# WU-CVGL/DreamMesh4D

Measured on AMD Instinct MI355X. Metric: rendered views/sec (fwd+bwd, 512^2, 200k Gaussians), higher is better.
Workload: dtype f32

## Files before the change

### dreammesh4d_amd/csrc/raster_preprocess.hip

```cpp
#include "common.h"
#include "raster.h"

#ifndef DM4D_GREC
#define DM4D_GREC 128
#endif
namespace dm4d {

struct f3 { float x, y, z; };

__device__ __forceinline__ f3 xform4x3(const f3 p, const float *M)
{
    f3 o;
    o.x = ((M[0] * p.x + M[4] * p.y) + M[8] * p.z) + M[12];
    o.y = ((M[1] * p.x + M[5] * p.y) + M[9] * p.z) + M[13];
    o.z = ((M[2] * p.x + M[6] * p.y) + M[10] * p.z) + M[14];
    return o;
}
__device__ __forceinline__ float4 xform4x4(const f3 p, const float *M)
{
    float4 o;
    o.x = ((M[0] * p.x + M[4] * p.y) + M[8] * p.z) + M[12];
    o.y = ((M[1] * p.x + M[5] * p.y) + M[9] * p.z) + M[13];
    o.z = ((M[2] * p.x + M[6] * p.y) + M[10] * p.z) + M[14];
    o.w = ((M[3] * p.x + M[7] * p.y) + M[11] * p.z) + M[15];
// ... 52 lines not shown
    float J02 = -(vp.focal_x * tcx) / (t.z * t.z);
    float J11 = vp.focal_y / t.z;
    float J12 = -(vp.focal_y * tcy) / (t.z * t.z);
    float T0[3], T1[3];
#pragma unroll
    for (int j = 0; j < 3; ++j) {
        T0[j] = J00 * V[j * 4 + 0] + J02 * V[j * 4 + 2];
        T1[j] = J11 * V[j * 4 + 1] + J12 * V[j * 4 + 2];
    }
    const float S[9] = {cov6[0], cov6[1], cov6[2], cov6[1], cov6[3], cov6[4], cov6[2], cov6[4], cov6[5]};
    float v0[3], v1[3];
#pragma unroll
    for (int j = 0; j < 3; ++j) {
        v0[j] = (T0[0] * S[0 * 3 + j] + T0[1] * S[1 * 3 + j]) + T0[2] * S[2 * 3 + j];
        v1[j] = (T1[0] * S[0 * 3 + j] + T1[1] * S[1 * 3 + j]) + T1[2] * S[2 * 3 + j];
    }
    c[0] = (v0[0] * T0[0] + v0[1] * T0[1]) + v0[2] * T0[2];
    c[1] = (v0[0] * T1[0] + v0[1] * T1[1]) + v0[2] * T1[2];
    c[2] = (v1[0] * T1[0] + v1[1] * T1[1]) + v1[2] * T1[2];
    if (aux) {
#pragma unroll
        for (int j = 0; j < 3; ++j) { aux->T0[j] = T0[j]; aux->T1[j] = T1[j]; }
        aux->tz = t.z;
        aux->tcx = tcx;
        aux->tcy = tcy;
        aux->xclamped = (txtz < -limx || txtz > limx);
        aux->yclamped = (tytz < -limy || tytz > limy);
    }
}

#define DM4D_SH_C0 0.28209479177387814f

__device__ __forceinline__ f3 load3(const float *p, int i) { return f3{p[3 * i], p[3 * i + 1], p[3 * i + 2]}; }

__global__ __launch_bounds__(kPreThreads) void k_preprocess(BatchDesc d)
{
    extern __shared__ __attribute__((aligned(16))) uint32_t s_hist[];
    const ViewCtx c = resolve(d, blockIdx.y);
    const ViewParams &vp = c.vp;
    const dm4d_raster_inputs &in = c.in;
    int32_t *__restrict__ radii = c.radii;
    const GeomPtrs &g = c.g;
    const int T = c.T;
    __shared__ float sV[16], sP[16];
    __shared__ uint32_t s_wsum[2][kPreThreads / 64];
    const int tid = threadIdx.x;
    if (tid < 16) { sV[tid] = vp.view[tid]; sP[tid] = vp.proj[tid]; }
    for (int t = tid; t < T; t += kPreThreads) s_hist[t] = 0u;
    __syncthreads();
    uint32_t touched_sum = 0, rec_sum = 0;
#pragma unroll 1
    for (int it = 0; it < kPreItems; ++it) {
        const int i = blockIdx.x * kPreBlock + it * kPreThreads + tid;
        if (i >= in.N) break;
        uint32_t touched = 0, recs = 0;
        int my_radius = 0;
        const f3 p = load3(in.means3D, i);
        const f3 pv = xform4x3(p, sV);
        if (pv.z > 0.2f) {
            const float4 ph = xform4x4(p, sP);
            const float pw = 1.0f / (ph.w + 0.0000001f);
            const float ppx = ph.x * pw, ppy = ph.y * pw;
            float cov6[6];
            if (in.cov3D_precomp) {
#pragma unroll
                for (int k = 0; k < 6; ++k) cov6[k] = in.cov3D_precomp[6 * (size_t)i + k];
            } else {
                const float4 q = reinterpret_cast<const float4 *>(in.rotations)[i];
                cov3d_from_scale_rot(load3(in.scales, i), vp.scale_modifier, q, cov6);
            }
            float c[3];
            cov2d(p, vp, sV, cov6, c, nullptr);
            c[0] += 0.3f;
            c[2] += 0.3f;
            const float det = c[0] * c[2] - c[1] * c[1];
            if (det != 0.0f) {
                const float det_inv = 1.f / det;
                const float mid = 0.5f * (c[0] + c[2]);
                const float disc = sqrtf(fmaxf(0.1f, mid * mid - det));
                const float lambda1 = mid + disc, lambda2 = mid - disc;
                const int r = f2i_sat(ceilf(3.f * sqrtf(fmaxf(lambda1, lambda2))));
                const float px = ((ppx + 1.0f) * (float)vp.W - 1.0f) * 0.5f;
                const float py = ((ppy + 1.0f) * (float)vp.H - 1.0f) * 0.5f;
                const Rect rc = tile_rect(px, py, r, vp.gx, vp.gy);
                const int area = (rc.x1 - rc.x0) * (rc.y1 - rc.y0);
                if (area != 0) {
                    my_radius = r;
                    touched = (uint32_t)area;
                    g.xy[i] = make_float2(px, py);
                    g.depth[i] = pv.z;
                    const float4 co = make_float4(c[2] * det_inv, -c[1] * det_inv, c[0] * det_inv, in.opacities[i]);
                    g.conic_opacity[i] = co;
                    const Bands bd = cell_bands(px, py, co.x, co.y, co.z, co.w, rc);
                    recs = (uint32_t)(bd.nbx * bd.nby);
                    uint32_t dense = 1u;
                    const float cdet = co.x * co.z - co.y * co.y;
                    if (bd.nbx >= 2 && bd.nby >= 2 && recs <= 64u && cdet > 0.f && co.x > 0.f && co.z > 0.f) {
                        const float tau = __logf(255.0f * co.w) * 1.001f + 0.01f;
                        const EllipseRows er = ellipse_rows(co.x, co.y, co.z, tau);
                        uint64_t mask = 0ull;
                        for (int by = 0; by < bd.nby; ++by) {
                            int b0, b1;
                            row_span(er, px, py, (float)(4 * (bd.by0 + by)), b0, b1);
                            b0 = max(b0 - bd.bx0, 0);
                            b1 = min(b1 - bd.bx0, bd.nbx - 1);
                            if (b0 <= b1) mask |= ((~0ull >> (63 - (b1 - b0))) << b0) << (by * bd.nbx);
                        }
                        g.cellmask[i] = mask;
                        recs = (uint32_t)__popcll(mask);
                        dense = 0u;
                    }
                    g.cellinfo[i] = make_uint4((uint32_t)bd.bx0 | ((uint32_t)bd.by0 << 16),
                                               (uint32_t)bd.nbx | ((uint32_t)bd.nby << 16), 0u, dense);
                    if (d.tile_records) {
                        const TileSpan ts = tile_span((uint32_t)bd.bx0 | ((uint32_t)bd.by0 << 16), (uint32_t)bd.nbx | ((uint32_t)bd.nby << 16));
                        recs = (uint32_t)(ts.tnx * ts.tny);
                    }
                    if (in.shs) {
                        const float *sh = in.shs + (size_t)i * in.sh_coeffs * 3;
#pragma unroll
                        for (int ch = 0; ch < 3; ++ch) {
                            float v = DM4D_SH_C0 * sh[ch] + 0.5f;
                            g.clamped[3 * (size_t)i + ch] = (v < 0.f);
                            g.rgb[3 * (size_t)i + ch] = fmaxf(v, 0.f);
                        }
                    }
                    for (int y = rc.y0; y < rc.y1; ++y)
                        for (int x = rc.x0; x < rc.x1; ++x) atomicAdd(&s_hist[y * vp.gx + x], 1u);
                }
            }
        }
        radii[i] = my_radius;
        g.tiles_touched[i] = touched;
        g.rec_touched[i] = recs;
        touched_sum += touched;
        rec_sum += recs;
    }
    const uint32_t ws = wave_sum_u32(touched_sum), wr = wave_sum_u32(rec_sum);
    if ((tid & 63) == 0) { s_wsum[0][tid >> 6] = ws; s_wsum[1][tid >> 6] = wr; }
    __syncthreads();
    uint32_t *row = g.hist + (size_t)blockIdx.x * T;
    for (int t = tid; t < T; t += kPreThreads) row[t] = s_hist[t];
    if (tid == 0) {
        uint32_t s = 0, r = 0;
#pragma unroll
        for (int w = 0; w < kPreThreads / 64; ++w) { s += s_wsum[0][w]; r += s_wsum[1][w]; }
        g.block_sums[blockIdx.x] = s;
        g.rec_block_sums[blockIdx.x] = r;
        if (s) atomicAdd(&g.counters[kCntD], s);
        if (r) atomicAdd(&g.counters[kCntR], r);
    }
}

__device__ __forceinline__ uint32_t block_excl_scan_256(uint32_t v, uint32_t *s_w , uint32_t *total)
{
    const int tid = threadIdx.x, lane = tid & 63, wv = tid >> 6;
    const uint32_t incl = wave_incl_scan_u32(v, lane);
    __syncthreads();
    if (lane == 63) s_w[wv] = incl;
    __syncthreads();
    uint32_t pre = 0, tot = 0;
#pragma unroll
    for (int w = 0; w < kPreThreads / 64; ++w) {
        const uint32_t x = s_w[w];
        if (w < wv) pre += x;
        tot += x;
    }
    *total = tot;
    return pre + incl - v;
}

__global__ __launch_bounds__(kPreThreads) void k_scatter(BatchDesc d)
{
    extern __shared__ __attribute__((aligned(16))) uint32_t s_cursor[];
    const ViewCtx c = resolve(d, blockIdx.y);
    const ViewParams &vp = c.vp;
    const int N = c.in.N, T = c.T;
    const int32_t *__restrict__ radii = c.radii;
    const GeomPtrs &g = c.g;
    const BinPtrs &b = c.b;
    const uint32_t cap = c.cap;
    __shared__ uint32_t s_w[kPreThreads / 64];
    const int tid = threadIdx.x;
    {
        const int per = (T + kPreThreads - 1) / kPreThreads;
        const int t0 = tid * per, t1 = min(T, t0 + per);
        uint32_t loc = 0;
        for (int t = t0; t < t1; ++t) loc += g.tile_count[t];
        uint32_t total;
        uint32_t run = block_excl_scan_256(loc, s_w, &total);
        const uint32_t *row = g.hist + (size_t)blockIdx.x * T;
        for (int t = t0; t < t1; ++t) {
            if (blockIdx.x == 0) g.tile_start[t] = run;
            s_cursor[t] = run + row[t];
            run += g.tile_count[t];
        }
        if (blockIdx.x == 0 && tid == 0) g.tile_start[T] = total;
    }
    if (blockIdx.x == 0) {
        __shared__ uint32_t s_oh[256], s_oc[256], s_omax;
        if (tid == 0) s_omax = 1u;
        s_oh[tid] = 0u;
        __syncthreads();
        uint32_t wmax = 0;
        for (int t = tid; t < T; t += kPreThreads) wmax = max(wmax, g.tile_count[t]);
        wmax = wave_max_u32(wmax);
        if ((tid & 63) == 0) atomicMax(&s_omax, wmax);
        __syncthreads();
        const float oscale = 255.0f / (float)s_omax;
        for (int t = tid; t < T; t += kPreThreads)
            atomicAdd(&s_oh[255 - min(255, (int)((float)g.tile_count[t] * oscale))], 1u);
        __syncthreads();
        if (tid == 0) {
            uint32_t run = 0;
            for (int k = 0; k < 256; ++k) { s_oc[k] = run; run += s_oh[k]; }
        }
        __syncthreads();
        for (int t = tid; t < T; t += kPreThreads)
            g.order[atomicAdd(&s_oc[255 - min(255, (int)((float)g.tile_count[t] * oscale))], 1u)] = (uint32_t)t;
    }
    uint32_t rcarry;
    {
        uint32_t rloc = 0;
        for (int w = tid; w < (int)blockIdx.x; w += kPreThreads) rloc += g.rec_block_sums[w];
        uint32_t total;
        block_excl_scan_256(rloc, s_w, &total);
        rcarry = total;
    }
    __syncthreads();
    bool overflow = false, rec_overflow = false;
#pragma unroll 1
    for (int it = 0; it < kPreItems; ++it) {
        const int i = blockIdx.x * kPreBlock + it * kPreThreads + tid;
        const uint32_t touched = (i < N) ? g.tiles_touched[i] : 0u;
        uint32_t total;
        const uint32_t recs = (i < N) ? g.rec_touched[i] : 0u;
        const uint32_t r0 = rcarry + block_excl_scan_256(recs, s_w, &total);
        rcarry += total;
        if (i < N && touched != 0u) {
            reinterpret_cast<uint32_t *>(g.cellinfo + i)[2] = r0;
            g.rec0[i] = r0;
            rec_overflow |= (recs > 0u) && ((uint64_t)r0 + recs > (uint64_t)c.rec_cap);
        }
        if (touched == 0) continue;
        const float2 xy = g.xy[i];
        const Rect rc = tile_rect(xy.x, xy.y, radii[i], vp.gx, vp.gy);
        const uint32_t dbits = __float_as_uint(g.depth[i]);
        uint32_t n = 0;
        for (int y = rc.y0; y < rc.y1; ++y)
            for (int x = rc.x0; x < rc.x1; ++x, ++n) {
                const uint32_t slot = atomicAdd(&s_cursor[y * vp.gx + x], 1u);
                if (slot < cap) {
                    b.u_depth[slot] = dbits;
                    b.u_idx[slot] = (uint32_t)i;
                } else {
                    overflow = true;
                }
            }
    }
    if (overflow) g.counters[kCntOverflow] = 1u;
    if (rec_overflow) g.counters[kCntRecOverflow] = 1u;
}

struct GatherOut { float dmean[3], drot[4], dcol[kMaxChannels]; };

constexpr int kGatherRecords(int parts) { return parts <= 3 ? DM4D_GREC : 96; }
template <int PARTS>
__device__ __forceinline__ void gather_gaussian(const BatchDesc &d, const ViewCtx &c, const int i, const bool live, const float *sV,
                                                const float *sP, float *chunk, GatherOut &res)
{
    const ViewParams &vp = c.vp;
    const dm4d_raster_inputs &in = c.in;
    const int32_t *__restrict__ radii = c.radii;
    const GeomPtrs &g = c.g;
    const float *__restrict__ dLt = c.dLq;
    const BwdOutputs &o = c.o;
    constexpr int kGRec = kGatherRecords(PARTS), kGStride = PARTS <= 3 ? 12 : 20;
    constexpr int NQ = kGRec * PARTS / 64;
    const int lane = threadIdx.x & 63;
    const size_t si = (size_t)i;
#pragma unroll
    for (int k = 0; k < 3; ++k) res.dmean[k] = 0.f;
#pragma unroll
    for (int k = 0; k < 4; ++k) res.drot[k] = 0.f;
#pragma unroll
    for (int k = 0; k < kMaxChannels; ++k) res.dcol[k] = 0.f;

    float acc[7 + kMaxChannels];
#pragma unroll
    for (int k = 0; k < 7 + kMaxChannels; ++k) acc[k] = 0.f;
    const int r = live ? radii[i] : 0;
    const int C = vp.C;
    f3 h_m = {0.f, 0.f, 0.f}, h_sc = {0.f, 0.f, 0.f};
    float4 h_q = make_float4(1.f, 0.f, 0.f, 0.f), h_co = make_float4(0.f, 0.f, 0.f, 0.f);
    if (r > 0) {
        h_m = load3(in.means3D, i);
        if (!in.cov3D_precomp) { h_q = reinterpret_cast<const float4 *>(in.rotations)[i]; h_sc = load3(in.scales, i); }
        h_co = g.conic_opacity[i];
    }
    {
        const bool lean = d.lean != 0;
        constexpr int RS = PARTS * 4;
        uint32_t rec0 = 0xFFFFFFFFu, end = 0u;
        if (r > 0) {
            const uint32_t cnt = g.rec_touched[i];
            if (cnt > 0u) {
                rec0 = g.cellinfo[i].z;
                end = min(rec0 + cnt, max(rec0, c.rec_cap));
            }
        }
        uint32_t R0 = rec0, R1 = end;
        R0 = wave_min_u32(R0);
        R1 = wave_max_u32(R1);
        float4 pq[NQ];
#pragma unroll
        for (int q = 0; q < NQ; ++q) pq[q] = make_float4(0.f, 0.f, 0.f, 0.f);
#define DM4D_FETCH(BASE)                                                                                   \
        {                                                                                                  \
            const uint32_t n4_ = min((uint32_t)kGRec, R1 - (BASE)) * (uint32_t)PARTS;                      \
            const float4 *src4_ = reinterpret_cast<const float4 *>(dLt + (size_t)(BASE) * RS);             \
            _Pragma("unroll") for (int q = 0; q < NQ; ++q)                                                 \
                if ((uint32_t)lane + 64u * q < n4_) pq[q] = src4_[lane + 64 * q];                          \
        }
        if (R0 < R1) DM4D_FETCH(R0)
        for (uint32_t base = R0; base < R1; base += kGRec) {
            const uint32_t nrec = min((uint32_t)kGRec, R1 - base);
            __builtin_amdgcn_wave_barrier();
#pragma unroll
            for (int q = 0; q < NQ; ++q) {
                const uint32_t idx4 = (uint32_t)lane + 64u * q;
                if (idx4 < nrec * (uint32_t)PARTS)
                    *reinterpret_cast<float4 *>(chunk + (idx4 / (uint32_t)PARTS) * kGStride + (idx4 % (uint32_t)PARTS) * 4) = pq[q];
            }
            if (base + kGRec < R1) DM4D_FETCH(base + kGRec)
            __builtin_amdgcn_wave_barrier();
            const uint32_t lo = max(rec0, base), hi = min(end, base + nrec);
            for (uint32_t slot = lo; slot < hi; ++slot) {
                const float4 *rp = reinterpret_cast<const float4 *>(chunk + (slot - base) * kGStride);
                const float4 a0 = rp[0], a1 = rp[1];
                acc[0] += a0.x; acc[1] += a0.y; acc[2] += a0.z; acc[3] += a0.w;
                if (PARTS == 2) {
                    acc[4] += a1.x; acc[10] += a1.y; acc[11] += a1.z; acc[12] += a1.w;
                    continue;
                }
                const float4 a2 = rp[2];
                if (lean) {
                    acc[4] += a1.x; acc[6] += a1.y; acc[10] += a1.z; acc[11] += a1.w; acc[12] += a2.x;
                    continue;
                }
                acc[4] += a1.x; acc[5] += a1.y; acc[6] += a1.z; acc[7] += a1.w;
                acc[8] += a2.x; acc[9] += a2.y;
                if (C > 3) {
                    const float4 a3 = rp[3];
                    acc[10] += a2.z; acc[11] += a2.w; acc[12] += a3.x;
                }
            }
        }
#undef DM4D_FETCH
    }
    {
        const float4 co = h_co;
        const float m0 = acc[0], m1 = acc[1];
        acc[0] = -(co.x * m0 + co.y * m1) * (0.5f * (float)vp.W);
        acc[1] = -(co.y * m0 + co.z * m1) * (0.5f * (float)vp.H);
        acc[2] = -0.5f * acc[2];
        acc[3] = -acc[3];
        acc[4] = -0.5f * acc[4];
    }
    if (!live) return;
    if (o.dL_dmeans2D) {
        o.dL_dmeans2D[3 * si + 0] = acc[0];
        o.dL_dmeans2D[3 * si + 1] = acc[1];
        o.dL_dmeans2D[3 * si + 2] = 0.f;
    }
#pragma unroll
    for (int ch = 0; ch < kMaxChannels; ++ch) res.dcol[ch] = acc[7 + ch];
    if (o.dL_dopacity) {
        const float op_ = in.opacities[i];
        o.dL_dopacity[si] = (r > 0 && op_ > 0.f) ? acc[5] / op_ : 0.f;
    }
    if (o.dL_dcolors) {
        for (int ch = 0; ch < C; ++ch) o.dL_dcolors[(size_t)C * si + ch] = acc[7 + ch];
    }
    if (o.dL_dsh && in.shs) {
        const int M = in.sh_coeffs;
        for (int ch = 0; ch < 3; ++ch)
            o.dL_dsh[si * M * 3 + ch] = (r > 0 && !g.clamped[3 * si + ch]) ? DM4D_SH_C0 * acc[7 + ch] : 0.f;
        for (int k = 3; k < 3 * M; ++k) o.dL_dsh[si * M * 3 + k] = 0.f;
    }

    float dmean[3] = {0.f, 0.f, 0.f};
    float dcov[6] = {0.f, 0.f, 0.f, 0.f, 0.f, 0.f};
    float dscale[3] = {0.f, 0.f, 0.f};
    float drot[4] = {0.f, 0.f, 0.f, 0.f};
    if (r > 0) {
        const f3 m = h_m;
        float cov6[6];
        float4 q = make_float4(1.f, 0.f, 0.f, 0.f);
        f3 sc = {0.f, 0.f, 0.f};
        if (in.cov3D_precomp) {
#pragma unroll
            for (int k = 0; k < 6; ++k) cov6[k] = in.cov3D_precomp[6 * si + k];
        } else {
            q = h_q; sc = h_sc;
            cov3d_from_scale_rot(sc, vp.scale_modifier, q, cov6);
        }
        float c[3];
        Cov2DAux aux;
        cov2d(m, vp, sV, cov6, c, &aux);
        const float a = c[0] + 0.3f, bb = c[1], cc = c[2] + 0.3f;
        const float denom = a * cc - bb * bb;
        const float denom2inv = 1.0f / ((denom * denom) + 0.0000001f);
        const float gA = acc[2], gB = acc[3], gC = acc[4];
        float dL_da = 0.f, dL_db = 0.f, dL_dc = 0.f;
        const float *T0 = aux.T0, *T1 = aux.T1;
        if (denom2inv != 0.f) {
            dL_da = denom2inv * (-cc * cc * gA + bb * cc * gB + (denom - a * cc) * gC);
            dL_dc = denom2inv * (-a * a * gC + a * bb * gB + (denom - a * cc) * gA);
            dL_db = denom2inv * (2 * bb * cc * gA - (denom + 2 * bb * bb) * gB + 2 * a * bb * gC);
            dcov[0] = T0[0] * T0[0] * dL_da + T0[0] * T1[0] * dL_db + T1[0] * T1[0] * dL_dc;
            dcov[3] = T0[1] * T0[1] * dL_da + T0[1] * T1[1] * dL_db + T1[1] * T1[1] * dL_dc;
            dcov[5] = T0[2] * T0[2] * dL_da + T0[2] * T1[2] * dL_db + T1[2] * T1[2] * dL_dc;
            dcov[1] = 2 * T0[0] * T0[1] * dL_da + (T0[0] * T1[1] + T0[1] * T1[0]) * dL_db + 2 * T1[0] * T1[1] * dL_dc;
            dcov[2] = 2 * T0[0] * T0[2] * dL_da + (T0[0] * T1[2] + T0[2] * T1[0]) * dL_db + 2 * T1[0] * T1[2] * dL_dc;
            dcov[4] = 2 * T0[2] * T0[1] * dL_da + (T0[1] * T1[2] + T0[2] * T1[1]) * dL_db + 2 * T1[1] * T1[2] * dL_dc;
        }
        {
            const float S[9] = {cov6[0], cov6[1], cov6[2], cov6[1], cov6[3], cov6[4], cov6[2], cov6[4], cov6[5]};
            float dT0[3], dT1[3];
#pragma unroll
            for (int k = 0; k < 3; ++k) {
                const float s0 = S[k * 3 + 0] * T0[0] + S[k * 3 + 1] * T0[1] + S[k * 3 + 2] * T0[2];
                const float s1 = S[k * 3 + 0] * T1[0] + S[k * 3 + 1] * T1[1] + S[k * 3 + 2] * T1[2];
                dT0[k] = 2 * s0 * dL_da + s1 * dL_db;
                dT1[k] = 2 * s1 * dL_dc + s0 * dL_db;
            }
            float dJ00 = 0, dJ02 = 0, dJ11 = 0, dJ12 = 0;
#pragma unroll
            for (int k = 0; k < 3; ++k) {
                dJ00 += sV[k * 4 + 0] * dT0[k];
                dJ02 += sV[k * 4 + 2] * dT0[k];
                dJ11 += sV[k * 4 + 1] * dT1[k];
                dJ12 += sV[k * 4 + 2] * dT1[k];
            }
            const float tz = 1.f / aux.tz, tz2 = tz * tz, tz3 = tz2 * tz;
            const float xm = aux.xclamped ? 0.f : 1.f, ym = aux.yclamped ? 0.f : 1.f;
            const float fx = vp.focal_x, fy = vp.focal_y;
            const float dtx = xm * -fx * tz2 * dJ02;
            const float dty = ym * -fy * tz2 * dJ12;
            const float dtz = -fx * tz2 * dJ00 - fy * tz2 * dJ11 + (2 * fx * aux.tcx) * tz3 * dJ02 +
                              (2 * fy * aux.tcy) * tz3 * dJ12;
#pragma unroll
            for (int j = 0; j < 3; ++j) dmean[j] = sV[j * 4 + 0] * dtx + sV[j * 4 + 1] * dty + sV[j * 4 + 2] * dtz;
        }
        {
            const float4 ph = xform4x4(m, sP);
            const float mw = 1.0f / (ph.w + 0.0000001f);
            const float mul1 = ph.x * mw * mw, mul2 = ph.y * mw * mw;
#pragma unroll
            for (int j = 0; j < 3; ++j)
                dmean[j] += (sP[j * 4 + 0] * mw - sP[j * 4 + 3] * mul1) * acc[0] +
                            (sP[j * 4 + 1] * mw - sP[j * 4 + 3] * mul2) * acc[1];
        }
        {
            const float mul3 = sV[2] * m.x + sV[6] * m.y + sV[10] * m.z + sV[14];
#pragma unroll
            for (int j = 0; j < 3; ++j) dmean[j] += (sV[j * 4 + 2] - sV[j * 4 + 3] * mul3) * acc[6];
        }
        if (!in.cov3D_precomp) {
            float R[9];
            quat_to_R(q, R);
            const float mod = vp.scale_modifier;
            const float s[3] = {mod * sc.x, mod * sc.y, mod * sc.z};
            const float Gs[9] = {dcov[0], 0.5f * dcov[1], 0.5f * dcov[2], 0.5f * dcov[1], dcov[3],
                                 0.5f * dcov[4], 0.5f * dcov[2], 0.5f * dcov[4], dcov[5]};
            float dR[9];
#pragma unroll
            for (int j = 0; j < 3; ++j) {
                float ds = 0.f;
#pragma unroll
                for (int aa = 0; aa < 3; ++aa) {
                    float a2 = 0.f;
#pragma unroll
                    for (int k = 0; k < 3; ++k) a2 += Gs[aa * 3 + k] * (R[k * 3 + j] * s[j]);
                    const float dM = 2.f * a2;
                    ds += R[aa * 3 + j] * dM;
                    dR[aa * 3 + j] = dM * s[j];
                }
                dscale[j] = mod * ds;
            }
            const float rr = q.x, x = q.y, y = q.z, z = q.w;
            drot[0] = 2 * (-z * dR[1] + y * dR[2] + z * dR[3] - x * dR[5] - y * dR[6] + x * dR[7]);
            drot[1] = 2 * (y * dR[1] + z * dR[2] + y * dR[3] - 2 * x * dR[4] - rr * dR[5] + z * dR[6] + rr * dR[7] - 2 * x * dR[8]);
            drot[2] = 2 * (-2 * y * dR[0] + x * dR[1] + rr * dR[2] + x * dR[3] + z * dR[5] - rr * dR[6] + z * dR[7] - 2 * y * dR[8]);
            drot[3] = 2 * (-2 * z * dR[0] - rr * dR[1] + x * dR[2] + rr * dR[3] - 2 * z * dR[4] + y * dR[5] + x * dR[6] + y * dR[7]);
        }
    }
#pragma unroll
    for (int k = 0; k < 3; ++k) res.dmean[k] = dmean[k];
#pragma unroll
    for (int k = 0; k < 4; ++k) res.drot[k] = drot[k];
    if (o.dL_dmeans3D) {
        o.dL_dmeans3D[3 * si + 0] = dmean[0];
        o.dL_dmeans3D[3 * si + 1] = dmean[1];
        o.dL_dmeans3D[3 * si + 2] = dmean[2];
    }
    if (o.dL_dcov3D) {
#pragma unroll
        for (int k = 0; k < 6; ++k) o.dL_dcov3D[6 * si + k] = dcov[k];
    }
    if (o.dL_dscales) {
        o.dL_dscales[3 * si + 0] = dscale[0];
        o.dL_dscales[3 * si + 1] = dscale[1];
        o.dL_dscales[3 * si + 2] = dscale[2];
    }
    if (o.dL_drotations)
        reinterpret_cast<float4 *>(o.dL_drotations)[i] = make_float4(drot[0], drot[1], drot[2], drot[3]);
}

constexpr int kGatherChunkFloats(int parts) { return kGatherRecords(parts) * (parts <= 3 ? 12 : 20); }
template <int PARTS>
__global__ __launch_bounds__(kPreThreads) void k_gather_bwd(BatchDesc d)
{
    const ViewCtx c = resolve(d, blockIdx.y);
    __shared__ float sV[16], sP[16];
    __shared__ __attribute__((aligned(16))) float s_chunk[kPreThreads / 64][kGatherChunkFloats(PARTS)];
    const int tid = threadIdx.x;
    if (tid < 16) { sV[tid] = c.vp.view[tid]; sP[tid] = c.vp.proj[tid]; }
    __syncthreads();
    const int i = blockIdx.x * kPreThreads + tid;
    GatherOut res;
    gather_gaussian<PARTS>(d, c, i, i < c.in.N, sV, sP, s_chunk[tid >> 6], res);
}

__global__ void k_mark_visible(int N, const float *__restrict__ means3D, const float *__restrict__ view,
                               uint8_t *__restrict__ present)
{
    const int i = blockIdx.x * blockDim.x + threadIdx.x;
    if (i >= N) return;
    const f3 pv = xform4x3(load3(means3D, i), view);
    present[i] = pv.z > 0.2f;
}

__global__ void k_zero_counters(BatchDesc d)
{
    const int b = blockIdx.x;
    if (threadIdx.x < 64) reinterpret_cast<uint32_t *>(d.geom + (size_t)b * d.geom_stride)[threadIdx.x] = 0u;
}

int launch_zero_counters(const BatchDesc &d, hipStream_t st)
{
    hipLaunchKernelGGL(k_zero_counters, dim3(d.B), dim3(64), 0, st, d);
    DM4D_HIP_CHECK(hipGetLastError());
    return DM4D_OK;
}

int launch_preprocess(const BatchDesc &d, hipStream_t st)
{
    const int nb = (d.N + kPreBlock - 1) / kPreBlock;
    if (nb == 0) return DM4D_OK;
    const int T = ((d.W + kTile - 1) / kTile) * ((d.H + kTile - 1) / kTile);
    if ((size_t)T * 4 > 32768)
        DM4D_HIP_CHECK(hipFuncSetAttribute((const void *)k_preprocess, hipFuncAttributeMaxDynamicSharedMemorySize, T * 4));
    ProfScope prof_(kKPreprocess, st);
    hipLaunchKernelGGL(k_preprocess, dim3(nb, d.B), dim3(kPreThreads), (size_t)T * 4, st, d);
    DM4D_HIP_CHECK(hipGetLastError());
    return DM4D_OK;
}

int launch_scatter(const BatchDesc &d, hipStream_t st)
{
    const int nb = (d.N + kPreBlock - 1) / kPreBlock;
    const int T = ((d.W + kTile - 1) / kTile) * ((d.H + kTile - 1) / kTile);
    if ((size_t)T * 4 > 32768)
        DM4D_HIP_CHECK(hipFuncSetAttribute((const void *)k_scatter, hipFuncAttributeMaxDynamicSharedMemorySize, T * 4));
    ProfScope prof_(kKScatter, st);
    hipLaunchKernelGGL(k_scatter, dim3(nb > 0 ? nb : 1, d.B), dim3(kPreThreads), (size_t)T * 4, st, d);
    DM4D_HIP_CHECK(hipGetLastError());
    return DM4D_OK;
}

int launch_gather_bwd(const BatchDesc &d, hipStream_t st)
{
    const int nb = (d.N + kPreThreads - 1) / kPreThreads;
    if (nb == 0) return DM4D_OK;
    ProfScope prof_(kKGatherBwd, st);
    if (grad_stride(d.C, d.lean) == 8) hipLaunchKernelGGL(k_gather_bwd<2>, dim3(nb, d.B), dim3(kPreThreads), 0, st, d);
    else if (grad_stride(d.C, d.lean) == 12) hipLaunchKernelGGL(k_gather_bwd<3>, dim3(nb, d.B), dim3(kPreThreads), 0, st, d);
    else hipLaunchKernelGGL(k_gather_bwd<4>, dim3(nb, d.B), dim3(kPreThreads), 0, st, d);
    DM4D_HIP_CHECK(hipGetLastError());
    return DM4D_OK;
}

int launch_mark_visible(int N, const float *means3D, const float *view, uint8_t *present, hipStream_t st)
{
    if (N <= 0) return DM4D_OK;
    hipLaunchKernelGGL(k_mark_visible, dim3((N + 255) / 256), dim3(256), 0, st, N, means3D, view, present);
    DM4D_HIP_CHECK(hipGetLastError());
    return DM4D_OK;
}

}
```

### dreammesh4d_amd/csrc/skinning.hip

```cpp
#include "common.h"
#include "raster.h"

namespace dm4d {

struct q4 { float x, y, z, w; };
struct v3 { float x, y, z; };

__device__ __forceinline__ v3 mk3(float x, float y, float z) { return v3{x, y, z}; }
__device__ __forceinline__ v3 operator+(v3 a, v3 b) { return v3{a.x + b.x, a.y + b.y, a.z + b.z}; }
__device__ __forceinline__ v3 operator-(v3 a, v3 b) { return v3{a.x - b.x, a.y - b.y, a.z - b.z}; }
__device__ __forceinline__ v3 operator*(float s, v3 a) { return v3{s * a.x, s * a.y, s * a.z}; }
__device__ __forceinline__ float dot(v3 a, v3 b) { return a.x * b.x + a.y * b.y + a.z * b.z; }
__device__ __forceinline__ v3 cross(v3 a, v3 b) { return v3{a.y * b.z - a.z * b.y, a.z * b.x - a.x * b.z, a.x * b.y - a.y * b.x}; }
__device__ __forceinline__ v3 ld3(const float *p, size_t i) { return v3{p[3 * i], p[3 * i + 1], p[3 * i + 2]}; }
__device__ __forceinline__ void st3(float *p, size_t i, v3 a) { p[3 * i] = a.x; p[3 * i + 1] = a.y; p[3 * i + 2] = a.z; }
__device__ __forceinline__ q4 ldq(const float *p, size_t i) { const float4 t = reinterpret_cast<const float4 *>(p)[i]; return q4{t.x, t.y, t.z, t.w}; }
__device__ __forceinline__ v3 qv(q4 q) { return v3{q.x, q.y, q.z}; }
__device__ __forceinline__ float qdot(q4 a, q4 b) { return a.x * b.x + a.y * b.y + a.z * b.z + a.w * b.w; }
__device__ __forceinline__ q4 qscale(float s, q4 a) { return q4{s * a.x, s * a.y, s * a.z, s * a.w}; }
__device__ __forceinline__ q4 qadd(q4 a, q4 b) { return q4{a.x + b.x, a.y + b.y, a.z + b.z, a.w + b.w}; }
__device__ __forceinline__ q4 qconj(q4 a) { return q4{-a.x, -a.y, -a.z, a.w}; }
__device__ __forceinline__ q4 qmul(q4 a, q4 b)
{
    return q4{a.w * b.x + a.x * b.w + a.y * b.z - a.z * b.y, a.w * b.y - a.x * b.z + a.y * b.w + a.z * b.x,
// ... 331 lines not shown
                     n.S[6] * p.x + n.S[7] * p.y + n.S[8] * p.z);
    const float qn = sqrtf(qdot(n.q, n.q));
    const q4 qr = qscale(1.f / qn, n.q);
    const q4 av = q4{0.5f * n.t.x, 0.5f * n.t.y, 0.5f * n.t.z, 0.f};
    v3 x_lbs = mk3(0, 0, 0);
    q4 br = q4{0, 0, 0, 0}, bd = q4{0, 0, 0, 0};
    if (a.method != kDqs) x_lbs = quad_sum3(w * (qact(n.q, y) + n.t));
    if (a.method != kLbs) {
        br = quad_sum4(qscale(w, qr));
        bd = quad_sum4(qscale(w, qmul(av, qr)));
    }
    const float eta_raw = quad_sum(w * n.o);
    const v3 rho = quad_sum3(w * so3_log(n.q));
    float eta = 1.f, g_eta = 0.f;
    v3 g_lbs = gx, g_dqs = mk3(0, 0, 0);
    q4 g_br = q4{0, 0, 0, 0}, g_bd = q4{0, 0, 0, 0};
    if (a.method != kLbs) {
        const float nn = sqrtf(qdot(br, br));
        const q4 rh = qscale(1.f / nn, br), dh = qscale(1.f / nn, bd);
        if (a.method == kDqs) { g_dqs = gx; g_lbs = mk3(0, 0, 0); }
        else {
            const v3 x_dqs = qact(rh, p) + qv(qmul(qscale(2.f, dh), qconj(rh)));
            eta = fminf(eta_raw + 0.4f, 1.0f);
            g_lbs = eta * gx;
            g_dqs = (1.f - eta) * gx;
            g_eta = (eta_raw + 0.4f < 1.0f) ? dot(gx, x_lbs - x_dqs) : 0.f;
        }
        q4 g_rh = a.pypose ? qact_grad_q_pp(rh, p, g_dqs) : qact_grad_q(rh, p, g_dqs);
        const q4 G = q4{g_dqs.x, g_dqs.y, g_dqs.z, 0.f};
        q4 g_dh, g_b;
        dqs_mul_grad(a.pypose, qscale(2.f, dh), qconj(rh), G, g_dh, g_b);
        g_dh = qscale(2.f, g_dh);
        g_rh = qadd(g_rh, q4{-g_b.x, -g_b.y, -g_b.z, g_b.w});
        g_bd = qscale(1.f / nn, g_dh);
        g_br = qadd(qscale(1.f / nn, g_rh), qscale(-(qdot(g_rh, rh) + qdot(g_dh, dh)) / nn, rh));
    }
    const v3 g_rho = a.pypose ? so3_exp_grad_pp(rho, gq) : so3_exp_grad(rho, gq);
    v3 g_t = mk3(0, 0, 0);
    q4 g_q = a.pypose ? so3_log_grad_pp(n.q, w * g_rho) : so3_log_grad(n.q, w * g_rho);
    float g_S[6] = {0, 0, 0, 0, 0, 0};
    if (a.method != kDqs) {
        const v3 h = w * g_lbs;
        g_t = g_t + h;
        g_q = qadd(g_q, a.pypose ? qact_grad_q_pp(n.q, y, h) : qact_grad_q(n.q, y, h));
        const v3 gy = qact_grad_p(n.q, h);
        g_S[0] = gy.x * p.x; g_S[1] = gy.y * p.y; g_S[2] = gy.z * p.z;
        g_S[3] = gy.x * p.y + gy.y * p.x;
        g_S[4] = gy.x * p.z + gy.z * p.x;
        g_S[5] = gy.y * p.z + gy.z * p.y;
    }
    if (a.method != kLbs) {
        const q4 g_d = qscale(w, g_bd);
        q4 g_a, g_qr;
        dqs_mul_grad(a.pypose, av, qr, g_d, g_a, g_qr);
        g_t = g_t + 0.5f * qv(g_a);
        g_qr = qadd(g_qr, qscale(w, g_br));
        g_q = qadd(g_q, qscale(1.f / qn, qadd(g_qr, qscale(-qdot(g_qr, qr), qr))));
    }
    const q4 g_p = qscale(1.f / n.pn, qadd(g_q, qscale(-qdot(g_q, n.q), n.q)));
    const float g_o = w * g_eta;
    if (!live) return;
    float *r = rec + ((size_t)v * 4 + k) * kNodeRec;
    r[0] = g_t.x; r[1] = g_t.y; r[2] = g_t.z;
    r[3] = g_p.x; r[4] = g_p.y; r[5] = g_p.z; r[6] = g_p.w;
    r[7] = g_S[0]; r[8] = g_S[1]; r[9] = g_S[2]; r[10] = g_S[3]; r[11] = g_S[4]; r[12] = g_S[5];
    r[13] = g_o * n.o * (1.f - n.o);
}

__global__ __launch_bounds__(64) void k_skin_bwd_node(int M, const int32_t *__restrict__ csr_off,
                                                      const int32_t *__restrict__ csr_item,
                                                      const float *__restrict__ rec, float *__restrict__ g_dx,
                                                      float *__restrict__ g_dr, float *__restrict__ g_ds,
                                                      float *__restrict__ g_do, size_t rec_view_stride)
{
    const int m = blockIdx.x, lane = threadIdx.x;
    if (m >= M) return;
    {
        const size_t bv = blockIdx.y, o = bv * M;
        rec += bv * rec_view_stride;
        if (g_dx) g_dx += o * 3;
        if (g_dr) g_dr += o * 4;
        if (g_ds) g_ds += o * 6;
        if (g_do) g_do += o;
    }
    float acc[kNodeRec];
#pragma unroll
    for (int i = 0; i < kNodeRec; ++i) acc[i] = 0.f;
    for (int e = csr_off[m] + lane; e < csr_off[m + 1]; e += 64) {
        const float *r = rec + (size_t)csr_item[e] * kNodeRec;
#pragma unroll
        for (int i = 0; i < kNodeRec; ++i) acc[i] += r[i];
    }
#pragma unroll
    for (int i = 0; i < kNodeRec; ++i) acc[i] = wave_sum_row3(acc[i]);
    if (lane != 63) return;
    if (g_dx) { g_dx[3 * m] = acc[0]; g_dx[3 * m + 1] = acc[1]; g_dx[3 * m + 2] = acc[2]; }
    if (g_dr) { g_dr[4 * m] = acc[3]; g_dr[4 * m + 1] = acc[4]; g_dr[4 * m + 2] = acc[5]; g_dr[4 * m + 3] = acc[6]; }
    if (g_ds) { for (int i = 0; i < 6; ++i) g_ds[6 * m + i] = acc[7 + i]; }
    if (g_do) g_do[m] = acc[13];
}

constexpr int kMaxPerFace = 6;
__constant__ float c_bary[4][kMaxPerFace][3] = {
    {{1.f / 3, 1.f / 3, 1.f / 3}},
    {{1.f / 2, 1.f / 4, 1.f / 4}, {1.f / 4, 1.f / 2, 1.f / 4}, {1.f / 4, 1.f / 4, 1.f / 2}},
    {{1.f / 3, 1.f / 3, 1.f / 3}, {2.f / 3, 1.f / 6, 1.f / 6}, {1.f / 6, 2.f / 3, 1.f / 6}, {1.f / 6, 1.f / 6, 2.f / 3}},
    {{2.f / 3, 1.f / 6, 1.f / 6}, {1.f / 6, 2.f / 3, 1.f / 6}, {1.f / 6, 1.f / 6, 2.f / 3},
     {1.f / 6, 5.f / 12, 5.f / 12}, {5.f / 12, 1.f / 6, 5.f / 12}, {5.f / 12, 5.f / 12, 1.f / 6}}};
__device__ __forceinline__ int bary_row(int G) { return G == 1 ? 0 : G == 3 ? 1 : G == 4 ? 2 : 3; }

__global__ __launch_bounds__(kSkinThreads) void k_face_fwd(int F, int G, int V, const int32_t *__restrict__ faces,
                                                           const float *__restrict__ vxyz,
                                                           const float *__restrict__ vrot,
                                                           const float *__restrict__ q_static ,
                                                           float *__restrict__ means, float *__restrict__ rots,
                                                           float *__restrict__ normals, int nstride,
                                                           const float *__restrict__ rgb, float *__restrict__ colors6, ZeroList zl)
{
    if (zl.n > 0 && blockIdx.x == 0 && blockIdx.y == 0)
        for (int t = threadIdx.x; t < zl.n * 64; t += kSkinThreads) reinterpret_cast<uint32_t *>(zl.base + (size_t)(t >> 6) * zl.stride)[t & 63] = 0u;
    const int i = blockIdx.x * kSkinThreads + threadIdx.x;
    if (i >= F * G) return;
    {
        const size_t bv = blockIdx.y, n = (size_t)F * G;
        vxyz += bv * V * 3;
        vrot += bv * V * 4;
        means += bv * n * 3;
        rots += bv * n * 4;
        if (normals) normals += bv * n * nstride;
        if (colors6) colors6 += bv * n * 6;
    }
    const int f = i / G, s = i - f * G;
    const int i0 = faces[3 * f], i1 = faces[3 * f + 1], i2 = faces[3 * f + 2];
    const float *b = c_bary[bary_row(G)][s];
    const v3 x0 = ld3(vxyz, i0), x1 = ld3(vxyz, i1), x2 = ld3(vxyz, i2);
    st3(means, i, (b[0] * x0 + b[1] * x1) + b[2] * x2);
    const v3 r = (b[0] * so3_log(ldq(vrot, i0)) + b[1] * so3_log(ldq(vrot, i1))) + b[2] * so3_log(ldq(vrot, i2));
    const q4 qd = so3_exp(r);
    const float4 qs = reinterpret_cast<const float4 *>(q_static)[i];
    const q4 Q = qmul(qd, q4{qs.y, qs.z, qs.w, qs.x});
    const float inv = 1.f / fmaxf(sqrtf(qdot(Q, Q)), 1e-12f);
    reinterpret_cast<float4 *>(rots)[i] = make_float4(Q.w * inv, Q.x * inv, Q.y * inv, Q.z * inv);
    if (normals) {
        const v3 c = cross(x1 - x0, x2 - x0);
        const v3 nn = (1.f / fmaxf(sqrtf(dot(c, c)), 1e-12f)) * c;
        float *o = normals + (size_t)i * nstride;
        o[0] = nn.x; o[1] = nn.y; o[2] = nn.z;
    }
    if (colors6) {
        float *o = colors6 + (size_t)i * 6;
        o[0] = rgb[3 * i]; o[1] = rgb[3 * i + 1]; o[2] = rgb[3 * i + 2];
    }
}

constexpr int kCornerRec = 6;
__device__ __forceinline__ void face_bwd_finish(const int F, const int G, const int32_t *__restrict__ faces,
                                                const float *__restrict__ vxyz, const float *__restrict__ vrot,
                                                const float *__restrict__ q_static, const bool has_means, const bool has_rots,
                                                const bool has_normals, const bool live, const int f, const int sl, const int base,
                                                const v3 gm, const q4 go, const v3 gn_in, float *__restrict__ rec, const int pypose,
                                                float (*s_log)[3] ,
                                                float (*s_val)[9] )
{
    const int tid = threadIdx.x;
    if (live && has_rots) {
        if (G >= 3) {
            if (sl < 3) {
                const v3 L = so3_log(ldq(vrot, faces[3 * f + sl]));
                s_log[base + sl][0] = L.x; s_log[base + sl][1] = L.y; s_log[base + sl][2] = L.z;
            }
        }
    }
    __syncthreads();
    if (live) {
        const size_t i = (size_t)f * G + sl;
        const float *b = c_bary[bary_row(G)][sl];
        v3 gr = mk3(0, 0, 0);
        if (has_rots) {
            v3 L0, L1, L2;
            if (G >= 3) {
                L0 = mk3(s_log[base][0], s_log[base][1], s_log[base][2]);
                L1 = mk3(s_log[base + 1][0], s_log[base + 1][1], s_log[base + 1][2]);
                L2 = mk3(s_log[base + 2][0], s_log[base + 2][1], s_log[base + 2][2]);
            } else {
                L0 = so3_log(ldq(vrot, faces[3 * f]));
                L1 = so3_log(ldq(vrot, faces[3 * f + 1]));
                L2 = so3_log(ldq(vrot, faces[3 * f + 2]));
            }
            const v3 r = (b[0] * L0 + b[1] * L1) + b[2] * L2;
            const q4 qd = so3_exp(r);
            const float4 qs4 = reinterpret_cast<const float4 *>(q_static)[i];
            const q4 qs = q4{qs4.y, qs4.z, qs4.w, qs4.x};
            const q4 Q = qmul(qd, qs);
            const float nq = fmaxf(sqrtf(qdot(Q, Q)), 1e-12f);
            const q4 out = qscale(1.f / nq, Q);
            const q4 gQ = qscale(1.f / nq, qadd(go, qscale(-qdot(go, out), out)));
            if (pypose) gr = so3_exp_grad_pp(r, gQ);
            else gr = so3_exp_grad(r, qmul(gQ, qconj(qs)));
        }
        float *o = s_val[tid];
        o[0] = gm.x; o[1] = gm.y; o[2] = gm.z; o[3] = gr.x; o[4] = gr.y; o[5] = gr.z; o[6] = gn_in.x; o[7] = gn_in.y; o[8] = gn_in.z;
    }
    __syncthreads();
    if (!live || sl != 0) return;
    v3 X[3] = {mk3(0, 0, 0), mk3(0, 0, 0), mk3(0, 0, 0)}, R[3] = {mk3(0, 0, 0), mk3(0, 0, 0), mk3(0, 0, 0)};
    v3 gn = mk3(0, 0, 0);
    for (int s2 = 0; s2 < G; ++s2) {
        const float *b = c_bary[bary_row(G)][s2];
        const float *o = s_val[base + s2];
        const v3 gm2 = mk3(o[0], o[1], o[2]), gr = mk3(o[3], o[4], o[5]);
        if (has_means) { X[0] = X[0] + b[0] * gm2; X[1] = X[1] + b[1] * gm2; X[2] = X[2] + b[2] * gm2; }
        if (has_rots) { R[0] = R[0] + b[0] * gr; R[1] = R[1] + b[1] * gr; R[2] = R[2] + b[2] * gr; }
        gn = gn + mk3(o[6], o[7], o[8]);
    }
    if (has_normals) {
        const int i0 = faces[3 * f], i1 = faces[3 * f + 1], i2 = faces[3 * f + 2];
        const v3 x0 = ld3(vxyz, i0), x1 = ld3(vxyz, i1), x2 = ld3(vxyz, i2);
        const v3 e1 = x1 - x0, e2 = x2 - x0, c = cross(e1, e2);
        const float cn = fmaxf(sqrtf(dot(c, c)), 1e-12f);
        const v3 nn = (1.f / cn) * c;
        const v3 gc = (1.f / cn) * (gn - dot(gn, nn) * nn);
        const v3 ge1 = cross(e2, gc), ge2 = cross(gc, e1);
        X[1] = X[1] + ge1;
        X[2] = X[2] + ge2;
        X[0] = X[0] - (ge1 + ge2);
    }
    float *o = rec + (size_t)f * 3 * kCornerRec;
#pragma unroll
    for (int j = 0; j < 3; ++j) {
        o[j * kCornerRec + 0] = X[j].x; o[j * kCornerRec + 1] = X[j].y; o[j * kCornerRec + 2] = X[j].z;
        o[j * kCornerRec + 3] = R[j].x; o[j * kCornerRec + 4] = R[j].y; o[j * kCornerRec + 5] = R[j].z;
    }
}

__global__ __launch_bounds__(kSkinThreads) void k_face_bwd_face(int F, int G, int V, const int32_t *__restrict__ faces,
                                                                const float *__restrict__ vxyz,
                                                                const float *__restrict__ vrot,
                                                                const float *__restrict__ q_static,
                                                                const float *__restrict__ g_means,
                                                                const float *__restrict__ g_rots,
                                                                const float *__restrict__ g_normals, int nstride,
                                                                float *__restrict__ rec ,
                                                                const int32_t *__restrict__ frame_index, int n_views, int pypose)
{
    const int tid = threadIdx.x;
    const int faces_per_wg = kSkinThreads / G;
    const int fl = tid / G, sl = tid - fl * G;
    const int f = blockIdx.x * faces_per_wg + fl;
    const bool live = fl < faces_per_wg && f < F;
    const size_t n = (size_t)F * G;
    const int frame = blockIdx.y;
    {
        const size_t bv = blockIdx.y;
        vxyz += bv * V * 3;
        vrot += bv * V * 4;
        rec += bv * F * 3 * kCornerRec;
    }
    const int b0 = frame_index ? 0 : frame, b1 = frame_index ? n_views : frame + 1;
    v3 gm = mk3(0, 0, 0), gn = mk3(0, 0, 0);
    q4 go = q4{0.f, 0.f, 0.f, 0.f};
    if (live) {
        const size_t i = (size_t)f * G + sl;
        for (int bv = b0; bv < b1; ++bv) {
            if (frame_index && frame_index[bv] != frame) continue;
            if (g_means) gm = gm + ld3(g_means + (size_t)bv * n * 3, i);
            if (g_rots) {
                const float4 go4 = reinterpret_cast<const float4 *>(g_rots + (size_t)bv * n * 4)[i];
                go = qadd(go, q4{go4.y, go4.z, go4.w, go4.x});
            }
            if (g_normals) {
                const float *pn = g_normals + ((size_t)bv * n + i) * nstride;
                gn = gn + mk3(pn[0], pn[1], pn[2]);
            }
        }
    }
    __shared__ float s_log[kSkinThreads][3];
    __shared__ float s_val[kSkinThreads][9];
    face_bwd_finish(F, G, faces, vxyz, vrot, q_static, g_means != nullptr, g_rots != nullptr, g_normals != nullptr, live, f, sl, fl * G,
                    gm, go, gn, rec, pypose, s_log, s_val);
}

__global__ __launch_bounds__(kSkinThreads) void k_face_bwd_vertex(int V, int F, const int32_t *__restrict__ csr_off,
                                                                  const int32_t *__restrict__ csr_item ,
                                                                  const float *__restrict__ vrot,
                                                                  const float *__restrict__ rec,
                                                                  const float *__restrict__ ext_xyz,
                                                                  const float *__restrict__ ext_rot,
                                                                  float *__restrict__ g_vxyz, float *__restrict__ g_vrot, int pypose,
                                                                  const int32_t *__restrict__ view_frame, int n_view_recs)
{
    const int gid = blockIdx.x * kSkinThreads + threadIdx.x;
    const int v = gid >> 3, c = gid & 7;
    const bool live = v < V;
    const int frame = blockIdx.y;
    {
        const size_t bv = blockIdx.y;
        vrot += bv * V * 4;
        if (n_view_recs <= 0) rec += bv * F * 3 * kCornerRec;
        g_vxyz += bv * V * 3;
        g_vrot += bv * V * 4;
        if (ext_xyz) ext_xyz += bv * V * 3;
        if (ext_rot) ext_rot += bv * V * 4;
    }
    float a[kCornerRec] = {0.f, 0.f, 0.f, 0.f, 0.f, 0.f};
    if (live) {
        const int nb = n_view_recs > 0 ? n_view_recs : 1;
        for (int b = 0; b < nb; ++b) {
            if (n_view_recs > 0 && (view_frame ? view_frame[b] : b) != frame) continue;
            const float *__restrict__ rb = rec + (n_view_recs > 0 ? (size_t)b * F * 3 * kCornerRec : 0);
            for (int e = csr_off[v] + c; e < csr_off[v + 1]; e += 8) {
                const float2 *r = reinterpret_cast<const float2 *>(rb + (size_t)csr_item[e] * kCornerRec);
                const float2 r0 = r[0], r1 = r[1], r2 = r[2];
                a[0] += r0.x; a[1] += r0.y; a[2] += r1.x; a[3] += r1.y; a[4] += r2.x; a[5] += r2.y;
            }
        }
    }
#pragma unroll
    for (int i = 0; i < kCornerRec; ++i) {
        a[i] = dpp_add<0xB1>(a[i]);
        a[i] = dpp_add<0x4E>(a[i]);
        a[i] = dpp_add<0x141>(a[i]);
    }
    if (!live || c != 0) return;
    v3 X = mk3(a[0], a[1], a[2]);
    if (ext_xyz) X = X + ld3(ext_xyz, v);
    st3(g_vxyz, v, X);
    q4 g = pypose ? so3_log_grad_pp(ldq(vrot, v), mk3(a[3], a[4], a[5])) : so3_log_grad(ldq(vrot, v), mk3(a[3], a[4], a[5]));
    if (ext_rot) g = qadd(g, ldq(ext_rot, v));
    reinterpret_cast<float4 *>(g_vrot)[v] = make_float4(g.x, g.y, g.z, g.w);
}

}

using namespace dm4d;

namespace dm4d {

int skin_forward_launch(int B, int method, int V, int M, int K, const float *verts, const int32_t *idx, const float *w,
                        const float *dx, const float *dr, const float *ds, const float *dop, float *out_xyz,
                        float *out_rot, hipStream_t st)
{
    if (V <= 0 || B <= 0) return DM4D_OK;
    method &= 0xff;
    SkinArgs a{method, V, M, K, 0, verts, idx, w, dx, dr, method == kDqs ? nullptr : ds, method == kHybrid ? dop : nullptr};
    ProfScope prof_(kKSkinFwd, st);
    hipLaunchKernelGGL(k_skin_fwd, dim3((V + kSkinThreads - 1) / kSkinThreads, B), dim3(kSkinThreads), 0, st, a, out_xyz, out_rot);
    DM4D_HIP_CHECK(hipGetLastError());
    return DM4D_OK;
}

int skin_backward_launch(int B, int method, int V, int M, int K, const float *verts, const int32_t *idx, const float *w,
                         const float *dx, const float *dr, const float *ds, const float *dop, const float *g_xyz,
                         const float *g_rot, const int32_t *csr_off, const int32_t *csr_items, float *scratch,
                         float *o_dx, float *o_dr, float *o_ds, float *o_do, hipStream_t st)
{
    if (B <= 0) return DM4D_OK;
    const int pypose = (method & kPypose) ? 1 : 0;
    method &= 0xff;
    SkinArgs a{method, V, M, K, pypose, verts, idx, w, dx, dr, method == kDqs ? nullptr : ds, method == kHybrid ? dop : nullptr};
    ProfScope prof_(kKSkinBwd, st);
    if (V > 0) {
        if (K == 4)
            hipLaunchKernelGGL(k_skin_bwd_vertex_k4, dim3((4 * V + kSkinThreads - 1) / kSkinThreads, B), dim3(kSkinThreads), 0, st, a,
                               g_xyz, g_rot, scratch);
        else
            hipLaunchKernelGGL(k_skin_bwd_vertex, dim3((V + kSkinThreads - 1) / kSkinThreads, B), dim3(kSkinThreads), 0, st, a,
                               g_xyz, g_rot, scratch);
        DM4D_HIP_CHECK(hipGetLastError());
    }
    hipLaunchKernelGGL(k_skin_bwd_node, dim3(M, B), dim3(64), 0, st, M, csr_off, csr_items,
                       (const float *)scratch, o_dx, o_dr, o_ds, o_do, (size_t)V * K * kNodeRec);
    DM4D_HIP_CHECK(hipGetLastError());
    return DM4D_OK;
}

int face_forward_launch(int B, int F, int G, int V, const int32_t *faces, const float *vxyz, const float *vrot,
                        const float *qs, float *means, float *rots, float *normals, int nstride, const float *rgb,
                        float *colors6, hipStream_t st, char *zero_base, size_t zero_stride, int zero_n)
{
    if (F <= 0 || B <= 0) return zero_n > 0 ? DM4D_ERR_INVALID : DM4D_OK;
    G &= 0xff;
    ProfScope prof_(kKFaceFwd, st);
    const ZeroList zl = {zero_base, zero_stride, zero_base ? zero_n : 0};
    hipLaunchKernelGGL(k_face_fwd, dim3((F * G + kSkinThreads - 1) / kSkinThreads, B), dim3(kSkinThreads), 0, st, F, G, V,
                       faces, vxyz, vrot, qs, means, rots, normals, nstride, rgb, colors6, zl);
    DM4D_HIP_CHECK(hipGetLastError());
    return DM4D_OK;
}

int face_backward_launch(int B, int F, int G, int V, const int32_t *faces, const float *vxyz, const float *vrot,
                         const float *qs, const float *g_means, const float *g_rots, const float *g_normals, int nstride,
                         const int32_t *csr_off, const int32_t *csr_items, float *scratch, const float *ext_xyz,
                         const float *ext_rot, float *o_vxyz, float *o_vrot, const int32_t *frame_index, int n_views,
                         hipStream_t st)
{
    if (B <= 0) return DM4D_OK;
    const int pypose = (G & kPypose) ? 1 : 0;
    G &= 0xff;
    ProfScope prof_(kKFaceBwd, st);
    if (F > 0 && !(n_views < 0)) {
        const int fpw = kSkinThreads / G;
        hipLaunchKernelGGL(k_face_bwd_face, dim3((F + fpw - 1) / fpw, B), dim3(kSkinThreads), 0, st, F, G,
                           V, faces, vxyz, vrot, qs, g_means, g_rots, g_normals, nstride, scratch, frame_index, n_views, pypose);
        DM4D_HIP_CHECK(hipGetLastError());
    }
    if (V > 0) {
        const int n_view_recs = n_views < -1 ? -n_views - 1 : 0;
        hipLaunchKernelGGL(k_face_bwd_vertex, dim3((8 * V + kSkinThreads - 1) / kSkinThreads, B), dim3(kSkinThreads), 0, st, V,
                           F, csr_off, csr_items, vrot, (const float *)scratch, ext_xyz, ext_rot, o_vxyz, o_vrot, pypose,
                           frame_index, n_view_recs);
        DM4D_HIP_CHECK(hipGetLastError());
    }
    return DM4D_OK;
}

int skin_check(int method, int V, int M, int K, const void *verts, const void *idx, const void *w, const void *dx,
               const void *dr, const void *ds, const void *dop)
{
    if ((method & ~kPypose) < 0 || (method & ~kPypose) > 2) { set_error("method must be 0 (lbs), 1 (dqs) or 2 (hybrid), optionally | DM4D_GRAD_PYPOSE"); return DM4D_ERR_INVALID; }
    method &= 0xff;
    if (V < 0 || M <= 0 || K <= 0 || K > kMaxK) { set_error("bad V/M/K (%d/%d/%d)", V, M, K); return DM4D_ERR_INVALID; }
    if (V > 0 && (!verts || !idx || !w || !dx || !dr)) { set_error("null input"); return DM4D_ERR_INVALID; }
    if (method != kDqs && !ds) { set_error("lbs/hybrid need the strain output ds"); return DM4D_ERR_INVALID; }
    if (method == kHybrid && !dop) { set_error("hybrid needs the opacity output"); return DM4D_ERR_INVALID; }
    return DM4D_OK;
}

int face_check(int F, int G, const void *faces, const void *vxyz, const void *vrot, const void *qs)
{
    G &= ~kPypose;
    if (F < 0 || !(G == 1 || G == 3 || G == 4 || G == 6)) { set_error("bad F/G (%d/%d); G must be 1, 3, 4 or 6", F, G); return DM4D_ERR_INVALID; }
    if (F > 0 && (!faces || !vxyz || !vrot || !qs)) { set_error("null input"); return DM4D_ERR_INVALID; }
    return DM4D_OK;
}

}

using namespace dm4d;

extern "C" {

int dm4d_skin_vertices_forward(int32_t method, int32_t V, int32_t M, int32_t K, const float *verts,
                               const int32_t *nbr_idx, const float *nbr_w, const float *dx, const float *dr,
                               const float *ds, const float *d_opacity, float *out_xyz, float *out_rot,
                               dm4d_stream_t stream)
{
    int rc = skin_check(method, V, M, K, verts, nbr_idx, nbr_w, dx, dr, ds, d_opacity);
    if (rc) return rc;
    if (V == 0) return DM4D_OK;
    if (!out_xyz || !out_rot) { set_error("null output"); return DM4D_ERR_INVALID; }
    return skin_forward_launch(1, method, V, M, K, verts, nbr_idx, nbr_w, dx, dr, ds, d_opacity, out_xyz, out_rot,
                               (hipStream_t)stream);
}

size_t dm4d_skin_scratch_bytes(int32_t V, int32_t K) { return (size_t)(V > 0 ? V : 1) * K * kNodeRec * 4; }

int dm4d_skin_vertices_backward(int32_t method, int32_t V, int32_t M, int32_t K, const float *verts,
                                const int32_t *nbr_idx, const float *nbr_w, const float *dx, const float *dr,
                                const float *ds, const float *d_opacity, const float *dL_dxyz, const float *dL_drot,
                                const int32_t *node_csr_offsets, const int32_t *node_csr_items, void *scratch,
                                float *dL_ddx, float *dL_ddr, float *dL_dds, float *dL_ddo, dm4d_stream_t stream)
{
    int rc = skin_check(method, V, M, K, verts, nbr_idx, nbr_w, dx, dr, ds, d_opacity);
    if (rc) return rc;
    if (!node_csr_offsets || !node_csr_items || !scratch) { set_error("null csr/scratch"); return DM4D_ERR_INVALID; }
    return skin_backward_launch(1, method, V, M, K, verts, nbr_idx, nbr_w, dx, dr, ds, d_opacity, dL_dxyz, dL_drot,
                                node_csr_offsets, node_csr_items, (float *)scratch, dL_ddx, dL_ddr, dL_dds, dL_ddo,
                                (hipStream_t)stream);
}

int dm4d_face_gaussians_forward(int32_t F, int32_t G, const int32_t *faces, const float *vxyz, const float *vrot,
                                const float *q_static_wxyz, float *means, float *rotations_wxyz, float *normals,
                                dm4d_stream_t stream)
{
    int rc = face_check(F, G, faces, vxyz, vrot, q_static_wxyz);
    if (rc) return rc;
    if (F == 0) return DM4D_OK;
    if (!means || !rotations_wxyz) { set_error("null output"); return DM4D_ERR_INVALID; }
    return face_forward_launch(1, F, G, 0, faces, vxyz, vrot, q_static_wxyz, means, rotations_wxyz, normals, 3, nullptr,
                               nullptr, (hipStream_t)stream, nullptr, 0, 0);
}

size_t dm4d_face_scratch_bytes(int32_t F) { return (size_t)(F > 0 ? F : 1) * 3 * kCornerRec * 4; }

int dm4d_face_gaussians_backward(int32_t F, int32_t G, int32_t V, const int32_t *faces, const float *vxyz,
                                 const float *vrot, const float *q_static_wxyz, const float *dL_dmeans,
                                 const float *dL_drotations_wxyz, const float *dL_dnormals,
                                 const int32_t *vert_csr_offsets, const int32_t *vert_csr_items, void *scratch,
                                 float *dL_dvxyz, float *dL_dvrot, dm4d_stream_t stream)
{
    int rc = face_check(F, G, faces, vxyz, vrot, q_static_wxyz);
    if (rc) return rc;
    if (V < 0 || !vert_csr_offsets || !vert_csr_items || !scratch || !dL_dvxyz || !dL_dvrot) { set_error("null csr/scratch/output"); return DM4D_ERR_INVALID; }
    return face_backward_launch(1, F, G, V, faces, vxyz, vrot, q_static_wxyz, dL_dmeans, dL_drotations_wxyz, dL_dnormals,
                                3, vert_csr_offsets, vert_csr_items, (float *)scratch, nullptr, nullptr, dL_dvxyz,
                                dL_dvrot, nullptr, 1, (hipStream_t)stream);
}

}
```

Before: 9994.

## Restructure skinning gradient gather with ballot view filtering and batched loads

The skinning backward gather now finds the views matching the current frame through a wave ballot, so lanes no longer each walk every view record. It processes up to four matching views and four CSR edges per step, issuing their loads together to expose memory-level parallelism. Per-vertex rotation and external gradients are prefetched before the loop. Separately, the raster preprocess backward reads the record start from a dedicated rec0 array instead of cellinfo.z and issues the loads without the radius branch. This adds register pressure and more complex control flow.

```diff
diff --git a/dreammesh4d_amd/csrc/raster_preprocess.hip b/dreammesh4d_amd/csrc/raster_preprocess.hip
--- a/dreammesh4d_amd/csrc/raster_preprocess.hip
+++ b/dreammesh4d_amd/csrc/raster_preprocess.hip
@@ -378,12 +378,11 @@
         const bool lean = d.lean != 0;
         constexpr int RS = PARTS * 4;
         uint32_t rec0 = 0xFFFFFFFFu, end = 0u;
-        if (r > 0) {
-            const uint32_t cnt = g.rec_touched[i];
-            if (cnt > 0u) {
-                rec0 = g.cellinfo[i].z;
-                end = min(rec0 + cnt, max(rec0, c.rec_cap));
-            }
+        const uint32_t cnt = live ? g.rec_touched[i] : 0u;
+        const uint32_t first = live ? g.rec0[i] : 0u;
+        if (r > 0 && cnt > 0u) {
+            rec0 = first;
+            end = min(rec0 + cnt, max(rec0, c.rec_cap));
         }
         uint32_t R0 = rec0, R1 = end;
         R0 = wave_min_u32(R0);
diff --git a/dreammesh4d_amd/csrc/skinning.hip b/dreammesh4d_amd/csrc/skinning.hip
--- a/dreammesh4d_amd/csrc/skinning.hip
+++ b/dreammesh4d_amd/csrc/skinning.hip
@@ -657,16 +657,71 @@
         if (ext_xyz) ext_xyz += bv * V * 3;
         if (ext_rot) ext_rot += bv * V * 4;
     }
+    const int lane = threadIdx.x & 63;
+    int e0 = 0, e1 = 0, it0 = 0;
+    q4 qv = q4{0.f, 0.f, 0.f, 0.f}, er = q4{0.f, 0.f, 0.f, 0.f};
+    v3 ex = mk3(0, 0, 0);
+    if (live) {
+        e0 = csr_off[v] + c;
+        e1 = csr_off[v + 1];
+        if (e0 < e1) it0 = csr_item[e0];
+        if (c == 0) {
+            qv = ldq(vrot, v);
+            if (ext_xyz) ex = ld3(ext_xyz, v);
+            if (ext_rot) er = ldq(ext_rot, v);
+        }
+    }
     float a[kCornerRec] = {0.f, 0.f, 0.f, 0.f, 0.f, 0.f};
-    if (live) {
-        const int nb = n_view_recs > 0 ? n_view_recs : 1;
-        for (int b = 0; b < nb; ++b) {
-            if (n_view_recs > 0 && (view_frame ? view_frame[b] : b) != frame) continue;
-            const float *__restrict__ rb = rec + (n_view_recs > 0 ? (size_t)b * F * 3 * kCornerRec : 0);
-            for (int e = csr_off[v] + c; e < csr_off[v + 1]; e += 8) {
-                const float2 *r = reinterpret_cast<const float2 *>(rb + (size_t)csr_item[e] * kCornerRec);
-                const float2 r0 = r[0], r1 = r[1], r2 = r[2];
-                a[0] += r0.x; a[1] += r0.y; a[2] += r1.x; a[3] += r1.y; a[4] += r2.x; a[5] += r2.y;
+    const int nb = n_view_recs > 0 ? n_view_recs : 1;
+    const size_t vstride = n_view_recs > 0 ? (size_t)F * 3 * kCornerRec : 0;
+    for (int bw = 0; bw < nb; bw += 64) {
+        const int bl = bw + lane;
+        const bool mine = bl < nb && (n_view_recs <= 0 || (view_frame ? view_frame[bl] : bl) == frame);
+        uint64_t m = __ballot(mine);
+        if (!live) continue;
+        constexpr int kVB = 4;
+        while (m) {
+            int vb[kVB];
+            int nv = 0;
+#pragma unroll
+            for (int k = 0; k < kVB; ++k) {
+                vb[k] = 0;
+                if (m) { vb[k] = bw + __builtin_ctzll(m); m &= m - 1; nv = k + 1; }
+            }
+            float2 r[kVB][3];
+#pragma unroll
+            for (int k = 0; k < kVB; ++k) {
+                if (k < nv && e0 < e1) {
+                    const float2 *p = reinterpret_cast<const float2 *>(rec + (size_t)vb[k] * vstride + (size_t)it0 * kCornerRec);
+                    r[k][0] = p[0]; r[k][1] = p[1]; r[k][2] = p[2];
+                }
+            }
+#pragma unroll
+            for (int k = 0; k < kVB; ++k) {
+                if (k >= nv || e0 >= e1) break;
+                a[0] += r[k][0].x; a[1] += r[k][0].y; a[2] += r[k][1].x; a[3] += r[k][1].y; a[4] += r[k][2].x; a[5] += r[k][2].y;
+                constexpr int kE = 4;
+                const float *__restrict__ rb = rec + (size_t)vb[k] * vstride;
+                for (int eb = e0 + 8; eb < e1; eb += 8 * kE) {
+                    int it[kE];
+#pragma unroll
+                    for (int j = 0; j < kE; ++j) it[j] = eb + 8 * j < e1 ? csr_item[eb + 8 * j] : 0;
+                    float2 q[kE][3];
+#pragma unroll
+                    for (int j = 0; j < kE; ++j) {
+                        if (eb + 8 * j < e1) {
+                            const float2 *p = reinterpret_cast<const float2 *>(rb + (size_t)it[j] * kCornerRec);
+                            q[j][0] = p[0]; q[j][1] = p[1]; q[j][2] = p[2];
+                        }
+                    }
+#pragma unroll
+                    for (int j = 0; j < kE; ++j) {
+                        if (eb + 8 * j < e1) {
+                            a[0] += q[j][0].x; a[1] += q[j][0].y; a[2] += q[j][1].x;
+                            a[3] += q[j][1].y; a[4] += q[j][2].x; a[5] += q[j][2].y;
+                        }
+                    }
+                }
             }
         }
     }
@@ -678,10 +733,10 @@
     }
     if (!live || c != 0) return;
     v3 X = mk3(a[0], a[1], a[2]);
-    if (ext_xyz) X = X + ld3(ext_xyz, v);
+    if (ext_xyz) X = X + ex;
     st3(g_vxyz, v, X);
-    q4 g = pypose ? so3_log_grad_pp(ldq(vrot, v), mk3(a[3], a[4], a[5])) : so3_log_grad(ldq(vrot, v), mk3(a[3], a[4], a[5]));
-    if (ext_rot) g = qadd(g, ldq(ext_rot, v));
+    q4 g = pypose ? so3_log_grad_pp(qv, mk3(a[3], a[4], a[5])) : so3_log_grad(qv, mk3(a[3], a[4], a[5]));
+    if (ext_rot) g = qadd(g, er);
     reinterpret_cast<float4 *>(g_vrot)[v] = make_float4(g.x, g.y, g.z, g.w);
 }
 
```

New measurement: 10020 (median of 6 runs). No clear change (+0.3%).
